# nmdp-bioinformatics/py-graph-imputation

Hardware: AMD Instinct MI355X
Metric: imputed subjects/sec (whole node), 5-locus CAU graph (higher is better)
Workload: dtype f64; 1 GPU; BASELINE configs[1]: CAU 5-locus graph, 10k synthetic fully-typed subjects; 10000 subjects per step and GPU, seed=rank; graph_nodes=35411, populations=1

## Files before the change

### py-graph-imputation_amd/csrc/grim_engine.hip

```cpp
#include <hip/hip_runtime.h>
#include <hip/hip_ext.h>
#include <stdio.h>
#include <stdlib.h>
#include <string.h>
#include <algorithm>
#include <atomic>
#include <mutex>
#include <string>
#include <vector>

#include "grim_plan_a.h"
#include "grim_plan_b.h"
#include "grim_small.h"
#include "grim_medium.h"
#include "grim_mid.h"
#include "grim_tables.h"
#include "grim_tokdev.h"
#include "grim_em.h"
#include "grim_engine_internal.h"
#include "grim_host_internal.h"
#include "grim_sdma.h"

__global__ __launch_bounds__(GRIM_WG, GRIM_WG_PER_CU) void grim_plan_a_kernel(DevArgs A) {
  __shared__ WgShared sh;
  __shared__ WaveTop wt[GRIM_NWAVE];
  const int tid = threadIdx.x;
  const int P = A.g.P;
  Slot S = make_slot(A, blockIdx.x);
  const uint32_t n_bail = A.bail_list ? A.queue[5] : 0, n_bail_heavy = A.bail_list ? A.queue[7] : 0;
  const uint32_t n_mid = A.mid_list ? A.queue[17] : 0;
  if (tid < GRIM_NWAVE * 4) ((unsigned long long *)sh.wctr)[tid] = 0;
  wg_arena(sh, wt);
// ... 186 lines not shown
  if (threadIdx.x == 0) pending = after_plan_b ? 0u : queue[2] + queue[6] + queue[9] + queue[10];
  for (int i = threadIdx.x; i < GRIM_NCTR + GRIM_NQ / 2; i += blockDim.x) host_state[i] = state[i];
  __syncthreads();
  if (pending) return;
  for (int i = threadIdx.x; i < GRIM_NCTR; i += blockDim.x) state[i] = 0;
  if (threadIdx.x < GRIM_NQ) ((uint32_t *)(state + GRIM_NCTR))[threadIdx.x] = threadIdx.x == 1 ? row_head0 : 0u;
}

struct grim_ctx {
  int device;
  hipStream_t stream;
  hipStream_t copy_stream;
  hipStream_t up_stream;
  GrimSdma *sdma;
  int export_mode;
  std::mutex err_mu;
  std::string err;
  std::mutex run_mu;
  int n_cu;
  void *scratch;
  uint64_t scratch_bytes;
  uint32_t *wctr;
  std::vector<grim_batch *> spare;
};

struct grim_graph {
  grim_ctx *ctx;
  DevGraph d;
  std::vector<void *> bufs;
  uint64_t bytes;
// ... 88 lines not shown
#define HIPCHK(call, ctxp, ret)                                                        \
  do {                                                                                 \
    hipError_t e_ = (call);                                                            \
    if (e_ != hipSuccess) {                                                            \
      set_err((ctxp), std::string(#call) + ": " + hipGetErrorString(e_));             \
      return ret;                                                                      \
    }                                                                                  \
  } while (0)

extern "C" int grim_device_count(void) {
  int n = 0;
  if (hipGetDeviceCount(&n) != hipSuccess) return 0;
  return n;
}

extern "C" grim_ctx *grim_create(int device_id) {
  int n = 0;
  if (hipGetDeviceCount(&n) != hipSuccess || n <= 0) {
    g_err = "grim_create: no HIP device visible";
    return nullptr;
  }
  if (device_id < 0 || device_id >= n) {
    g_err = "grim_create: device id out of range";
    return nullptr;
  }
  grim_ctx *c = new grim_ctx();
  c->device = device_id;
  c->copy_stream = nullptr;
  c->up_stream = nullptr;
  if (hipSetDevice(device_id) != hipSuccess || hipStreamCreate(&c->stream) != hipSuccess ||
// ... 8 lines not shown
  c->scratch = nullptr;
  c->scratch_bytes = 0;
  c->wctr = nullptr;
  if (hipMalloc((void **)&c->wctr, 4 * GRIM_WCTR_WORDS) != hipSuccess) {
    (void)hipGetLastError();
    g_err = "grim_create: cannot allocate the work counters";
    hipStreamDestroy(c->stream);
    hipStreamDestroy(c->copy_stream);
    hipStreamDestroy(c->up_stream);
    delete c;
    return nullptr;
  }
  if (hipGetDeviceProperties(&prop, device_id) == hipSuccess) c->n_cu = prop.multiProcessorCount;
  c->sdma = nullptr;
  c->export_mode = 1;
  {
    const char *e = getenv("GRIM_EXPORT");
    int want = 2;
    if (e && !strcmp(e, "kernel")) want = 1;
    else if (e && !strcmp(e, "memcpy")) want = 0;
    else if (!e && getenv("GRIM_EXPORT_KERNEL")) want = atoi(getenv("GRIM_EXPORT_KERNEL")) ? 1 : 0;
    if (want == 2) {
      char bdf[64] = {0};
      const char *why = nullptr;
      if (hipDeviceGetPCIBusId(bdf, (int)sizeof(bdf), device_id) != hipSuccess) bdf[0] = 0;
      c->sdma = grim_sdma_open(bdf[0] ? bdf : nullptr, device_id, &why);
      if (c->sdma) {
        const size_t probe = 1500000;
        void *hp = nullptr, *dp = nullptr;
        char report[256];
// ... 176 lines not shown
static uint64_t align256(uint64_t x) { return (x + 255) & ~255ull; }

static thread_local int tl_device = -1;
static inline void use_device(int dev) {
  if (tl_device != dev) {
    hipSetDevice(dev);
    tl_device = dev;
  }
}

static int env_int(const char *name, int dflt) {
  const char *v = getenv(name);
  return v ? atoi(v) : dflt;
}

uint32_t engine_small_stride(const grim_params *p) { return GRIM_SMALL_ROWS_FIXED + (p->n_results < 16 ? p->n_results : 16); }

uint64_t engine_rows_per_subject(const grim_params *p, uint32_t P) {
  return 2ull * p->n_results + 2ull * (p->n_pop_results < (uint64_t)P * P ? p->n_pop_results : (uint64_t)P * P);
}

static bool dev_realloc(uint8_t *&ptr, uint64_t bytes) {
  if (ptr) hipFree(ptr);
  ptr = nullptr;
  return hipMalloc((void **)&ptr, bytes ? bytes : 256) == hipSuccess;
}
static bool pin_realloc(uint8_t *&ptr, uint64_t bytes) {
  if (ptr) hipHostFree(ptr);
  ptr = nullptr;
  return hipHostMalloc((void **)&ptr, bytes ? bytes : 256, hipHostMallocDefault) == hipSuccess;
}
// ... 370 lines not shown
  }
  b->dev_lo = ld->dev_lo;
  b->dev_hi = ld->dev_hi;
  b->n_dev_lines = ld->dev_hi > ld->dev_lo ? ld->dev_hi - ld->dev_lo : 0;
  b->n_irregular = 0;
  b->n_subj = ld->n_subj;
  b->n_small = ld->n_small;
  b->n_medium = ld->n_medium;
  b->n_general = ld->n_general;
  b->last_load = *ld;
  b->last_load.priors = nullptr;
  A.n_medium = ld->n_medium;
  A.n_work = ld->n_general;
  unsigned long long *hs = (unsigned long long *)b->h_in;
  memset(hs, 0, 8 * (GRIM_NCTR + GRIM_NQ / 2));
  {
    const uint64_t staged = ((uint64_t)b->n_small + b->n_dev_lines) * b->small_stride;
    A.row_cap = (uint32_t)(b->row_limit - (staged <= b->row_limit ? staged : 0));
  }
  const bool host_subjects = ld->n_small + ld->n_medium + ld->n_general > 0;
  const uint64_t bytes = (!host_subjects && b->n_dev_lines) ? b->off_subj : b->off_tok + 2 * ld->tok_used;
  HIPCHK(hipMemcpyAsync(b->d_in, b->h_in, bytes, hipMemcpyHostToDevice, c->up_stream), c, -1);
  HIPCHK(hipEventRecord(b->ev_up, c->up_stream), c, -1);
  b->up_pending = true;
  g_moved[0] += bytes;
  {
    uint64_t R = (1ull << 20) + 512ull * ((uint64_t)ld->n_medium + ld->n_general) + 16ull * ld->n_small;
    R += (uint64_t)(ld->n_general < 256u ? ld->n_general : 256u) * (A.pair_cap / 2);
    const char *env_pool = getenv("GRIM_PAIR_POOL");
    if (env_pool && atol(env_pool) > 0) R = (uint64_t)atol(env_pool);
    if (b->pool_want > R) R = b->pool_want;
    if (R > 0x7FFFFFF0ull) R = 0x7FFFFFF0ull;
    const uint64_t items = 2ull * ld->n_subj < R / 256 + 1 ? 2ull * ld->n_subj : R / 256 + 1;
    uint64_t cap_b = R / 4 + (items + 1) * ((uint64_t)P * P + 4), cap_u = R / 4 + items * 64 + 1024;
// ... 17 lines not shown
    }
    b->pool_cap = R;
    A.ppool = (PairRec *)(b->d_pool + o_pool);
    A.ppool_cap = (uint32_t)R;
    A.taux = (TabAux *)(b->d_pool + o_aux);
    A.tboff = (uint32_t *)(b->d_pool + o_boff);
    A.tcell = (CellRec *)(b->d_pool + o_cell);
    A.tboff_cap = (uint32_t)cap_b;
    A.tunits = (TabUnit *)(b->d_pool + o_units);
    A.tunits_cap = (uint32_t)cap_u;
    A.tstride = (uint32_t)R;
    A.psort = (uint32_t *)(b->d_pool + o_sort);
    A.pgrp = (GrpRec *)(b->d_pool + o_grp);
    A.pprob = (double *)(b->d_pool + o_prob);
  }
  const uint32_t per_block = GRIM_WG / 32;
  b->n_host_small_waves = ((b->n_small + per_block - 1) / per_block) * (GRIM_WG / 64);
  b->n_small_waves = b->n_host_small_waves + ((b->n_dev_lines + per_block - 1) / per_block) * (GRIM_WG / 64);
  uint32_t slots = (uint32_t)c->n_cu * GRIM_WG_PER_CU;
  static const int env_slots = env_int("GRIM_SLOTS", 0);
  if (env_slots > 0) slots = (uint32_t)env_slots;
  if (slots > ld->n_subj) slots = ld->n_subj;
  if (slots == 0) slots = 1;
  b->n_slots = slots;
  b->scratch_need = (uint64_t)A.lay.stride * slots;
  if (b->gexec) {
    hipGraphExecDestroy(b->gexec);
    b->gexec = nullptr;
  }
  b->graph_state = 0;
  b->rows_used = 0;
  b->small_ctr_pending = false;
  return 0;
// ... 122 lines not shown
  launch(b, PH_NONE, grim_tables_merge_wave_kernel, dim3(g5), dim3(64), A);
  launch_span(b, PH_TABLES, false, true, grim_tables_merge_kernel, dim3(g2), dim3(GRIM_WG), A);
}

static void enqueue_half_wave(grim_batch *b, bool timed, const DevArgs &Ak, const SmallRec *recs, const uint32_t *order, uint32_t n, uint32_t stage) {
  const uint32_t per_block = GRIM_WG / 32;
  launch(b, timed ? PH_HALF_WAVE : PH_NONE, grim_plan_a_small_kernel, dim3((n + per_block - 1) / per_block), dim3(GRIM_WG), Ak, recs, n, stage,
         b->small_stride);
  launch(b, timed ? PH_COMPACT : PH_NONE, grim_small_compact_kernel, dim3((n + 63) / 64), dim3(64), b->a, order, order ? nullptr : recs, n, stage,
         b->small_stride);
}

static int enqueue_stage1(grim_batch *b) {
  grim_ctx *c = b->ctx;
  DevArgs &A = b->a;
  const uint32_t stage0 = (uint32_t)b->row_limit - (b->n_small + b->n_dev_lines) * b->small_stride;
  if (b->n_small) enqueue_half_wave(b, b->n_dev_lines == 0, A, b->d_small, b->d_os, b->n_small, stage0);
  if (b->n_dev_lines) {
    DevTok T;
    T.text = b->d_text;
    T.lines = b->d_lines;
    T.lo = b->dev_lo;
    T.hi = b->dev_hi;
    T.dict = b->dict->d;
    T.dsmall = b->d_dsmall;
    T.subj = const_cast<grim_subject *>(A.subj);
    T.tok = const_cast<uint16_t *>(A.tok);
    T.tok_base = (uint32_t)(b->plan.tok_cap ? b->plan.tok_cap : 1);
    T.graph_loci = A.g.n_loci;
    const dim3 tgrid((b->n_dev_lines + (GRIM_WG / 64) * TOK_LINES_PER_WAVE - 1) / ((GRIM_WG / 64) * TOK_LINES_PER_WAVE));
    launch(b, PH_TOKENIZER, grim_tokenize_kernel, tgrid, dim3(GRIM_WG), A, T);
    DevArgs A2 = A;
    A2.small_ctr = A.small_ctr + 2 * b->n_host_small_waves;
    enqueue_half_wave(b, true, A2, b->d_dsmall, nullptr, b->n_dev_lines, stage0 + b->n_small * b->small_stride);
  }
  if (b->n_medium) {
    static const int waves_per_cu = env_int("GRIM_MEDIUM_WAVES", GRIM_MEDIUM_WAVES_PER_CU);
    uint32_t grid = (uint32_t)c->n_cu * (uint32_t)(waves_per_cu > 0 ? waves_per_cu : GRIM_MEDIUM_WAVES_PER_CU);
    if (grid > b->n_medium) grid = b->n_medium;
    launch(b, PH_ONE_WAVE, grim_plan_a_medium_kernel, dim3(grid), dim3(64), A, b->d_om, b->n_medium, A.bail_list);
  }
  if (A.mid_list && b->n_general + b->n_medium) {
    const uint32_t want = b->n_general + b->n_medium;
    uint32_t grid = (uint32_t)c->n_cu * GRIM_MID_WG_PER_CU;
    if (grid > want) grid = want;
    launch(b, PH_MID, grim_plan_a_mid_kernel, dim3(grid), dim3(GRIM_WG), A);
  }
  if (b->n_general + b->n_medium) {
    uint32_t want = b->n_general + b->n_medium;
// ... 11 lines not shown
  return 0;
}

int engine_batch_upload_done(grim_batch *b) {
  if (!b || !b->up_pending) return 1;
  use_device(b->ctx->device);
  if (hipEventQuery(b->ev_up) == hipSuccess) return 1;
  (void)hipGetLastError();
  return 0;
}

int engine_batch_enqueue(grim_batch *b) {
  if (!b) return -1;
  grim_ctx *c = b->ctx;
  use_device(c->device);
  if (((uint64_t)b->n_small + b->n_dev_lines) * b->small_stride > b->row_limit) {
    b->rows_used = 0;
    set_err(c, "grim_batch_run: output row pool smaller than the half-wave kernel's fixed region");
    return -2;
  }
  memset(b->ms, 0, sizeof(b->ms));
  b->launched = 0;
  std::lock_guard<std::mutex> lk(c->run_mu);
  if (bind_scratch(b) != 0) return -1;
  if (b->up_pending) {
    b->up_pending = false;
    if (hipEventQuery(b->ev_up) != hipSuccess) {
      (void)hipGetLastError();
      HIPCHK(hipStreamWaitEvent(c->stream, b->ev_up, 0), c, -1);
    }
  }
  if (b->timing) {
    if (enqueue_stage1(b) != 0) {
      set_err(c, "grim_batch_run: kernel launch failed");
      return -1;
// ... 616 lines not shown
```

### py-graph-imputation_amd/csrc/grim_layout.h

```cpp
#pragma once
#include <stdint.h>

#include "../../include/grim_hip.h"

struct SmallRec {
  uint16_t tok[2 * GRIM_MAXL];
  uint8_t slot[GRIM_MAXL];
  uint8_t same;
  uint16_t prior_idx;
  uint32_t si;
};

struct PairRec {
  uint64_t k1, k2;
  double prob;
  uint32_t e1, e2;
};

struct TabWork {
  uint32_t si, n, off, mask;
};
#define GRIM_TAB_T1_MAX 256
struct TabAux {
  uint32_t boff[2];
// ... 7 lines not shown
  double sum;
  uint32_t head, pad;
};
struct CellRec {
  double sum;
  uint32_t first, pad;
};
struct TabUnit {
  uint32_t item, tb;
  uint32_t off;
  uint32_t lo, n;
  uint32_t pad[3];
};

#define GRIM_SMALL_ROWS_FIXED 1

enum { GRIM_CLS_SMALL = 0, GRIM_CLS_MEDIUM = 1, GRIM_CLS_GENERAL = 2 };

struct ClassRule {
  bool small_ok;
  bool medium_ok;
  double medium_max_cost;
  uint32_t graph_loci;
  uint64_t opt_threshold;
};

static inline double grim_cost(const grim_subject &sj);
static inline int grim_classify(const ClassRule &R, const grim_subject &sj) {
  bool sm = R.small_ok && sj.n_loci == GRIM_MAXL && R.graph_loci == GRIM_MAXL && sj.flags == 0;
  for (int l = 0; l < GRIM_MAXL && sm; ++l) sm = sj.cnt[l][0] == 1 && sj.cnt[l][1] == 1 && sj.wid[l][0] == 1 && sj.wid[l][1] == 1;
// ... 30 lines not shown
```

### py-graph-imputation_amd/csrc/grim_small.h

```cpp
#pragma once
#include "grim_pair.h"


__device__ __forceinline__ double half_shfl_d(double v, int src_in_half) {
  return __shfl(v, (threadIdx.x & 32) | src_in_half);
}
__device__ __forceinline__ uint32_t half_shfl_u(uint32_t v, int src_in_half) {
  return __shfl(v, (threadIdx.x & 32) | src_in_half);
}

template <int CTRL>
__device__ __forceinline__ double dpp_d(double v) {
  const long long b = __double_as_longlong(v);
  const int lo = __builtin_amdgcn_update_dpp(0, (int)(uint32_t)b, CTRL, 0xF, 0xF, false);
  const int hi = __builtin_amdgcn_update_dpp(0, (int)(uint32_t)((unsigned long long)b >> 32), CTRL, 0xF, 0xF, false);
  return __longlong_as_double((long long)(((unsigned long long)(uint32_t)hi << 32) | (uint32_t)lo));
}
__device__ __forceinline__ double row16_max(double v) {
  double o;
  o = dpp_d<0x121>(v); v = o > v ? o : v;
  o = dpp_d<0x122>(v); v = o > v ? o : v;
  o = dpp_d<0x124>(v); v = o > v ? o : v;
  o = dpp_d<0x128>(v); v = o > v ? o : v;
  return v;
}

__global__ __launch_bounds__(GRIM_WG) void grim_plan_a_small_kernel(DevArgs A, const SmallRec *recs, uint32_t n,
                                                                   uint32_t row_base, uint32_t row_stride) {
  const DevGraph &g = A.g;
  const int hl = threadIdx.x & 31;
  const uint32_t w = blockIdx.x * (GRIM_WG / 32) + (threadIdx.x >> 5);
  bool live = w < n;
  const int n_ladder = A.prm.n_ladder;
  double lad[8];
#pragma unroll
  for (int i = 0; i < 8; ++i) lad[i] = A.prm.ladder[i];
  bool hit = false;
  uint64_t mykey = 0;
  double f = 0.0;
  uint32_t same = 0, si = 0;
  double w_prior = 0.0;
  if (live) {
    const uint4 *rp = (const uint4 *)(recs + w);
    const uint4 r0 = rp[0], r1 = rp[1];
    const uint32_t words[8] = {r0.x, r0.y, r0.z, r0.w, r1.x, r1.y, r1.z, r1.w};
    same = (words[6] >> 8) & 0xFFu;
    si = words[7];
    live = si != GRIM_NONE;
    w_prior = live ? A.priors[(uint64_t)(words[6] >> 16)] : 0.0;
#pragma unroll
    for (int l = 0; l < GRIM_MAXL; ++l) {
      const uint32_t tw = words[l];
      const uint32_t t = ((hl >> l) & 1) ? (tw >> 16) : (tw & 0xFFFFu);
      const uint32_t slot = (l < 4 ? (words[5] >> (8 * l)) : words[6]) & 0xFFu;
      mykey |= (uint64_t)(t + 1u) << (GRIM_ABITS * slot);
    }
    uint32_t h = fht_hash(mykey) & g.fht_mask;
    for (; live;) {
      const FullEnt e = g.fht[h];
      if (e.key == mykey) { hit = true; f = e.f0; break; }
      if (e.key == 0) break;
      h = (h + 1) & g.fht_mask;
    }
  }
  const bool hit2 = half_shfl_u(hit ? 1u : 0u, hl ^ 31) != 0;
  const double f2 = half_shfl_d(f, hl ^ 31);
  const uint64_t key2 = ((uint64_t)half_shfl_u((uint32_t)(mykey >> 32), hl ^ 31) << 32) | half_shfl_u((uint32_t)mykey, hl ^ 31);
  const uint32_t het4 = 15u & ~same;
  bool kept = hl < 16 && ((uint32_t)hl & ~het4 & 15u) == 0 && (!((same >> 4) & 1u) || ((uint32_t)hl ^ het4) >= (uint32_t)hl);
  const bool pair_ok = live && kept && f > 0.0 && f2 > 0.0;
  const bool same_hap = mykey == key2;
  PairRef pr;
  pr.p1 = f; pr.p2 = f2; pr.m2 = f2;
  pr.e1 = same_hap ? 0u : 1u; pr.e2 = 0u;
  const bool hi_half = (threadIdx.x & 32) != 0;
  double eps = 0.0;
  bool found = false;
// ... 1 lines not shown
  {
    const uint64_t okb = __ballot(pair_ok);
    bool need_lo = (okb & 0xFFFFull) != 0, need_hi = ((okb >> 32) & 0xFFFFull) != 0;
    bool got_lo = false, got_hi = false;
    double eps_lo = 0.0, eps_hi = 0.0;
    auto step = [&](double e) {
      const bool a = pair_ok && pair_accept(e, pr, w_prior);
      const uint64_t b = __ballot(a);
      const bool take_lo = need_lo && (b & 0xFFFFull), take_hi = need_hi && ((b >> 32) & 0xFFFFull);
      if (take_lo) { need_lo = false; got_lo = true; eps_lo = e; }
      if (take_hi) { need_hi = false; got_hi = true; eps_hi = e; }
      if (hi_half ? take_hi : take_lo) acc = a;
    };
#pragma unroll
    for (int idx = 0; idx < 8; ++idx)
      if (idx < n_ladder && (need_lo || need_hi)) step(lad[idx]);
    for (int idx = 8; idx < n_ladder && (need_lo || need_hi); ++idx) step(A.prm.ladder[idx]);
    eps = hi_half ? eps_hi : eps_lo;
    found = hi_half ? got_hi : got_lo;
  }
  double prob = acc ? pair_prob(pr, w_prior) : 0.0;
  double mx = row16_max(prob);
  if (found && eps > 0.0) {
    eps = mx / 100000.0;
    acc = pair_ok && pair_accept(eps, pr, w_prior);
    prob = acc ? pair_prob(pr, w_prior) : 0.0;
    mx = row16_max(prob);
  }
  const uint64_t bal = __ballot(acc);
  const uint32_t accmask = (uint32_t)(hi_half ? (bal >> 32) : bal) & 0xFFFFu;
  const uint32_t nU = __popc(accmask);
  double total = 0.0;
  bool first = true;
  uint32_t rank = 0;
  for (uint32_t um = ((uint32_t)bal | (uint32_t)(bal >> 32)) & 0xFFFFu; um; um &= um - 1) {
    const int i = __builtin_ctz(um);
    const double p_lo = lane_get(prob, i), p_hi = lane_get(prob, 32 + i);
    const double pi = hi_half ? p_hi : p_lo;
    if ((accmask >> i) & 1u) {
      total = first ? pi : total + pi;
      first = false;
      if (pi > prob || (pi == prob && i < hl)) ++rank;
    }
  }
  {
    const uint64_t need = __ballot(live && kept), needp = __ballot(live && kept && hit),
                   needq = __ballot(live && kept && hit2);
    if ((threadIdx.x & 63) == 0) {
      const uint32_t gw = blockIdx.x * (GRIM_WG / 64) + (threadIdx.x >> 6);
      *(uint2 *)(A.small_ctr + 2 * gw) = make_uint2(2u * (uint32_t)__popcll(need), (uint32_t)(__popcll(needp) + __popcll(needq)));
    }
  }
  if (!live) return;
  const uint32_t off = row_base + w * row_stride;
  const bool ok = nU > 0;
  const int first_lane = ok ? (__ffs(accmask) - 1) : 0;
  const uint32_t n_pm = (ok && A.prm.out_haps) ? (nU < A.prm.n_results ? nU : A.prm.n_results) : 0;
  const uint64_t ka = ((uint64_t)half_shfl_u((uint32_t)(mykey >> 32), first_lane) << 32) | half_shfl_u((uint32_t)mykey, first_lane);
  const uint64_t kb = ((uint64_t)half_shfl_u((uint32_t)(key2 >> 32), first_lane) << 32) | half_shfl_u((uint32_t)key2, first_lane);
  {
    const int f = hl - 16;
    const bool phase = hl < 16;
    const bool wr = ok && (phase ? (acc && rank < n_pm) : f == 0);
    if (wr) {
      grim_row r;
      r.a = phase ? mykey : ka;
      r.b = phase ? key2 : kb;
      r.prob = phase ? prob : total;
      r.popa = 0;
      r.popb = 0;
      A.rows[off + (phase ? GRIM_SMALL_ROWS_FIXED + rank : (uint32_t)f)] = r;
    }
  }
  if (hl >= 19 && hl < 26) {
    const int j = hl - 19;
    const uint8_t status = ok ? GRIM_ST_OK : (A.prm.planb ? GRIM_ST_UNSUPPORTED : GRIM_ST_MISS);
    const uint32_t head = (uint32_t)status | ((uint32_t)'a' << 8) | ((!ok && A.prm.planb) ? (2u << 16) : 0u);
    const uint32_t n_um = (ok && A.prm.out_muug && A.prm.n_results) ? 1u : 0u;
    const uint32_t n_up = (ok && A.prm.out_muug && A.prm.n_pop_results) ? 1u : 0u;
    const uint32_t n_pp = (ok && A.prm.out_haps && A.prm.n_pop_results) ? 1u : 0u;
    const uint64_t mxb = ok ? (uint64_t)__double_as_longlong(mx) : 0ull;
    uint32_t lo, hi;
    switch (j) {
      case 0: lo = head; hi = ok ? nU : 0u; break;
      case 1: lo = ok ? 1u : 0u; hi = ok ? off + 0 : 0u; break;
      case 2: lo = ok ? off + 0 : 0u; hi = ok ? off + GRIM_SMALL_ROWS_FIXED : 0u; break;
      case 3: lo = ok ? off + 0 : 0u; hi = n_um; break;
      case 4: lo = n_up; hi = n_pm; break;
      case 5: lo = n_pp; hi = 0u; break;
      default: lo = (uint32_t)mxb; hi = (uint32_t)(mxb >> 32); break;
    }
    ((uint2 *)(A.res + si))[j] = make_uint2(lo, hi);
  }
  if (!ok && hl == 0 && A.prm.planb) push_next(A, si, false);
}
```

### py-graph-imputation_amd/csrc/grim_stream.cpp

```cpp
#include <errno.h>
#include <execinfo.h>
#include <fcntl.h>
#include <signal.h>
#include <sched.h>
#include <hip/hip_runtime_api.h>
#include <stdint.h>
#include <stdio.h>
#include <stdlib.h>
#include <string.h>
#include <sys/stat.h>
#include <sys/types.h>
#include <unistd.h>
#if defined(__x86_64__)
#include <immintrin.h>
#endif

#include <algorithm>
#include <atomic>
#include <chrono>
#include <condition_variable>
#include <deque>
#include <memory>
#include <mutex>
#include <string>
// ... 147 lines not shown
  grim_ctx *ctx = nullptr;
  const grim_graph *graph = nullptr;
  grim_params prm;
  grim_stream_opts opt;
  DictSnap snap;
  StreamRaces races;
  MaskTable masks;
  bool have_masks = false;
  ClassRule rule;
  FmtParams fp;
  uint32_t n_pops = 0;
  uint32_t chunk_lines = 0, granule = 1024, n_threads = 1, depth = 0;
  uint64_t rows_per_chunk = 0;
  grim_devdict *devdict = nullptr;
  bool dev_tok = false;
  std::atomic<uint64_t> rows_hint{0};
  uint64_t rows_max = 0;
  std::atomic<uint64_t> pool_hint{0};
  uint32_t cur_segment = 0;
  std::vector<std::array<uint64_t, 7>> seg_end;
  std::vector<uint8_t> seg_set;
  struct SegBuf {
    int k;
    char *p;
    size_t n;
    uint64_t rel;
  };
  struct PlacedWrite {
    int k;
    char *p;
// ... 185 lines not shown
      ld.text_bytes = c->text.size();
    }
    static const double one = 1.0;
    if (!s->races.n) {
      ld.n_priors = 0;
      ld.priors = &one;
    }
    lrc = engine_batch_load(b, &ld);
  }
  g_dbg_ns[0] += (uint64_t)(secs(tp0, tp1) * 1e9);
  g_dbg_ns[1] += (uint64_t)(secs(tp1, Clock::now()) * 1e9);
  return lrc;
}

static void part_stats(grim_stream *s, grim_batch *b, PartStats &ps) {
  if (!s->opt.timing) return;
  static_assert(sizeof(ps.kernel_ms) == sizeof(grim_stream_stats::kernel_ms), "kernel_ms: seven slots, GRIM_MS_TOTAL .. GRIM_MS_TABLES");
  for (int w = GRIM_MS_TOTAL; w <= GRIM_MS_TABLES; ++w) ps.kernel_ms[w] += grim_batch_kernel_ms(b, w);
  uint64_t ctr[4];
  if (grim_batch_counters(b, ctr) == 0)
    for (int k = 0; k < 4; ++k) ps.counters[k] += ctr[k];
}

static int device_part_sync(grim_stream *s, Chunk *c, uint32_t lo, uint32_t hi, bool whole, PartStats &ps);

static int fixup_part(grim_stream *s, Chunk *c, uint32_t lo, uint32_t hi, PartStats &ps) {
  grim_batch *b = c->batch;
  const uint32_t nrows1 = grim_batch_total_rows(b);
  const size_t base1 = c->extra_rows.size();
  c->extra_rows.resize(base1 + nrows1);
  if (engine_batch_fetch(b, lo, hi, nrows1 ? c->extra_rows.data() + base1 : nullptr) != 0) return -1;
  const EngineHost *H = engine_batch_host(b);
  grim_subject_result *res = H->res;
// ... 1233 lines not shown
  s->chunk_lines = opts->chunk_lines ? opts->chunk_lines : 131072u;
  s->granule = 1024;
  if (s->chunk_lines < s->granule) s->granule = s->chunk_lines;
  s->depth = opts->depth ? opts->depth : 4u;
  int nt = opts->n_threads;
  if (nt <= 0) nt = (int)grim_default_threads();
  s->n_threads = (uint32_t)nt;
  const uint64_t per = engine_rows_per_subject(prm, n_pops);
  uint64_t rows = opts->rows_per_chunk ? opts->rows_per_chunk : 32ull * s->chunk_lines;
  const uint64_t floor_rows = 2ull * engine_small_stride(prm) * s->chunk_lines + 2 * per + 4 * 64 + 1024;
  if (rows < floor_rows && !(opts->rows_exact && opts->rows_per_chunk)) rows = floor_rows;
  if (rows > 0x7FFFFFF0ull) rows = 0x7FFFFFF0ull;
  s->rows_per_chunk = rows;
  s->rows_max = opts->rows_per_chunk ? 0 : std::max<uint64_t>(rows, std::min<uint64_t>(0x7FFFFFF0ull, floor_rows + per * s->chunk_lines));
  {
    const char *e = getenv("GRIM_DEVICE_TOKENIZER");
    s->dev_tok = s->rule.small_ok && !s->have_masks && s->snap.n_loci == GRIM_MAXL && !(e && atoi(e) == 0);
    if (s->dev_tok) {
      s->devdict = engine_devdict_create(ctx, &s->snap);
      if (!s->devdict) {
        delete s;
        return nullptr;
      }
    }
  }
  EnginePlan plan0{s->chunk_lines, (uint64_t)s->chunk_lines * 48, s->dev_tok ? (uint64_t)s->chunk_lines * 128 : 0ull};
  for (uint32_t i = 0; i < s->depth; ++i) {
    std::unique_ptr<Chunk> c(new Chunk());
    c->slot_no = (int)i;
    c->batch = engine_batch_create(ctx, g, prm, rows, &plan0);
// ... 98 lines not shown
```

### py-graph-imputation_amd/csrc/grim_tokdev.h

```cpp
#pragma once
#include "grim_dev.h"
#include "grim_tok.h"

struct DevTok {
  const uint8_t *text;
  const LineRec *lines;
  uint32_t lo, hi;
  DevDict dict;
  SmallRec *dsmall;
  grim_subject *subj;
  uint16_t *tok;
  uint32_t tok_base;
  uint32_t graph_loci;
};
#define GRIM_REASON_HOST_TOKENIZER 7
#define GRIM_Q_IRREGULAR 18

#define TOK_LANES (2 * GRIM_MAXL)
#define TOK_LINES_PER_WAVE (64 / TOK_LANES)

__global__ __launch_bounds__(GRIM_WG) void grim_tokenize_kernel(DevArgs A, DevTok T) {
  const int lane = lane_id();
  const int a = lane % TOK_LANES, lw = lane / TOK_LANES;
  const uint32_t idx = (blockIdx.x * (GRIM_WG / 64) + wave_id()) * TOK_LINES_PER_WAVE + lw;
  const uint32_t line = T.lo + idx;
  const bool in_grid = lw < TOK_LINES_PER_WAVE && line < T.hi;
  LineRec lr;
  lr.gl_off = 0; lr.gl_len = 0; lr.prior_idx = 0;
  if (in_grid) lr = T.lines[line];
  const bool active = in_grid && lr.gl_len != 0;
  bool bad = active && lr.gl_len > GRIM_TOK_MAXGL;
  const uint32_t n = (active && !bad) ? lr.gl_len : 0;
  __shared__ uint4 lbuf[GRIM_WG / 64][TOK_LINES_PER_WAVE + 1][TOK_LANES];
  uint4 *mybuf = lbuf[wave_id()][lw < TOK_LINES_PER_WAVE ? lw : TOK_LINES_PER_WAVE];
  const uint32_t a0 = lr.gl_off & ~15u, skip = lr.gl_off - a0, tot = n ? skip + n : 0;
  uint4 q = make_uint4(0, 0, 0, 0);
  if (16u * (uint32_t)a < tot) q = ((const uint4 *)(T.text + a0))[a];
  mybuf[a] = q;
  uint32_t m_sep = 0, m_plus = 0;
  {
    const uint32_t wd[4] = {q.x, q.y, q.z, q.w};
#pragma unroll
    for (int bb = 0; bb < 16; ++bb) {
      const uint32_t pos = 16u * (uint32_t)a + (uint32_t)bb;
      const uint32_t c = (wd[bb >> 2] >> (8 * (bb & 3))) & 0xFFu;
      const bool in = pos >= skip && pos < tot;
      if (in && c == '+') m_plus |= 1u << bb;
      if (in && (c == '+' || c == '^')) m_sep |= 1u << bb;
// ... 98 lines not shown
    for (int k = 0; k < GRIM_MAXL; ++k) {
      const int src = base + 2 * k;
      const int sk = __shfl(slot, src < 64 ? src : 0);
      const int ek = __shfl(eq ? 1 : 0, src < 64 ? src : 0);
      if (sk >= 0) {
        used |= 1u << sk;
        slots5 |= (uint32_t)sk << (4 * k);
      }
      same |= (uint32_t)(ek & 1) << k;
    }
  }
  const uint64_t badm = __ballot(bad);
  const uint32_t line_bad = (uint32_t)(badm >> base) & ((1u << TOK_LANES) - 1u);
  const bool ok = active && line_bad == 0 && __popc(used) == GRIM_MAXL && T.graph_loci == GRIM_MAXL && T.dict.n_loci == GRIM_MAXL;
  if (!in_grid) return;
  SmallRec *rec = T.dsmall + idx;
  if (ok) {
    rec->tok[a] = (uint16_t)id;
    T.tok[(uint64_t)T.tok_base + (uint64_t)TOK_LANES * line + a] = (uint16_t)id;
    if ((a & 1) == 0) rec->slot[a >> 1] = (uint8_t)slot;
  }
  if (a == 0) {
    if (ok) {
      rec->same = (uint8_t)same;
      rec->prior_idx = lr.prior_idx;
      rec->si = line;
      grim_subject sj;
      sj.tok_off = T.tok_base + TOK_LANES * line;
      sj.prior_idx = lr.prior_idx;
      sj.n_loci = GRIM_MAXL;
      sj.flags = 0;
// ... 5 lines not shown
      }
      sj.pad[0] = (uint8_t)same;
      sj.pad[1] = sj.pad[2] = 0;
      sj.reserved[0] = sj.reserved[1] = 0;
      T.subj[line] = sj;
    } else {
      rec->si = GRIM_NONE;
      if (active) {
        uint32_t *r = (uint32_t *)(A.res + line);
        r[0] = (uint32_t)GRIM_ST_UNSUPPORTED | ((uint32_t)'a' << 8) | ((uint32_t)GRIM_REASON_HOST_TOKENIZER << 16);
        atomicAdd(A.queue + GRIM_Q_IRREGULAR, 1u);
      }
    }
  }
}
```

Before: 180.6 million subjects/s.

## Fuse device tokenizer and small-subject scoring into one chunk kernel

Adds a fused kernel that tokenizes device lines into LDS records, scores them in the same workgroup with the first hash-table probe issued early for all rounds, and writes rows compactly via a workgroup prefix sum and one atomic row reservation. This replaces the separate tokenize kernel plus half-wave small kernel, removing a launch and the global round-trip of SmallRec records, and no longer reserves a fixed per-subject staging stride for device lines. It adds an atomic on the row head per workgroup and a larger LDS footprint that may lower occupancy. It is enabled by default but disabled when timing is on.

```diff
diff --git a/py-graph-imputation_amd/csrc/grim_chunk.h b/py-graph-imputation_amd/csrc/grim_chunk.h
--- /dev/null
+++ b/py-graph-imputation_amd/csrc/grim_chunk.h
@@ -0,0 +1,97 @@
+#pragma once
+#include "grim_small.h"
+#include "grim_tokdev.h"
+
+#define CHUNK_ROUNDS (TOK_LINES_PER_WAVE / 2)
+#define CHUNK_ROWS_MAX (GRIM_SMALL_ROWS_FIXED + GRIM_SMALL_PM_MAX)
+#define CHUNK_HDR_PIECES ((int)(sizeof(grim_subject_result) / 8))
+#define CHUNK_COPY_LANES (GRIM_WG / TOK_LINES_PER_WG)
+
+struct ChunkShared {
+  TokLineBuf lbuf[GRIM_WG / 64];
+  SmallRec rec[TOK_LINES_PER_WG];
+  grim_row rows[TOK_LINES_PER_WG][CHUNK_ROWS_MAX];
+  uint2 hdr[TOK_LINES_PER_WG][CHUNK_HDR_PIECES];
+  uint32_t cnt[TOK_LINES_PER_WG];
+  uint32_t pre[TOK_LINES_PER_WG];
+  uint32_t base;
+  uint32_t fits;
+};
+static_assert(TOK_LINES_PER_WAVE % 2 == 0, "a round is two records");
+static_assert(TOK_LINES_PER_WG <= 64, "one wave takes the prefix over the workgroup's row counts");
+static_assert(sizeof(SmallRec) == 32 && sizeof(grim_row) == 32 && sizeof(grim_subject_result) == 8 * 7, "layouts the copies below rely on");
+static_assert(offsetof(ChunkShared, rec) % 16 == 0 && offsetof(ChunkShared, rows) % 16 == 0, "16-byte LDS reads");
+static_assert(sizeof(ChunkShared) <= 24 * 1024, "several workgroups per CU");
+
+__global__ __launch_bounds__(GRIM_WG) void grim_chunk_kernel(DevArgs A, DevTok T) {
+  __shared__ ChunkShared sh;
+  const int tid = threadIdx.x, wv = wave_id(), lane = lane_id();
+  const SmallLadder L = small_ladder(A);
+  if (lane < TOK_LINES_PER_WAVE) sh.rec[wv * TOK_LINES_PER_WAVE + lane].si = GRIM_NONE;
+  tokenize_block(A, T, sh.rec, sh.lbuf);
+  WAVE_SYNC();
+  const int half = (tid >> 5) & 1, hl = tid & 31;
+  SmallCand c[CHUNK_ROUNDS];
+  FullEnt e[CHUNK_ROUNDS];
+#pragma unroll
+  for (int r = 0; r < CHUNK_ROUNDS; ++r) c[r] = small_key(A, &sh.rec[wv * TOK_LINES_PER_WAVE + 2 * r + half], true);
+#pragma unroll
+  for (int r = 0; r < CHUNK_ROUNDS; ++r) {
+    e[r].key = 0;
+    e[r].f0 = 0.0;
+    if (c[r].live) e[r] = A.g.fht[c[r].h];
+  }
+  uint32_t probes = 0, hits = 0;
+#pragma unroll
+  for (int r = 0; r < CHUNK_ROUNDS; ++r) {
+    const int k = wv * TOK_LINES_PER_WAVE + 2 * r + half;
+    const SmallOut o = small_score(A, L, c[r], e[r], sh.rows[k], sh.hdr[k], 0u);
+    probes += o.probes;
+    hits += o.hits;
+    if (hl == 0) sh.cnt[k] = o.n_rows;
+  }
+  if (lane == 0) *(uint2 *)(A.small_ctr + 2 * (blockIdx.x * (GRIM_WG / 64) + wv)) = make_uint2(probes, hits);
+  __syncthreads();
+  if (wv == 0) {
+    const uint32_t n = lane < TOK_LINES_PER_WG ? sh.cnt[lane] : 0u;
+    uint32_t incl = n;
+    for (int d = 1; d < 64; d <<= 1) {
+      const uint32_t o = __shfl_up(incl, d);
+      if (lane >= d) incl += o;
+    }
+    if (lane < TOK_LINES_PER_WG) sh.pre[lane] = incl - n;
+    if (lane == 63) {
+      const uint32_t total = incl;
+      uint32_t base = 0, fits = 1;
+      if (total) {
+        base = atomicAdd(A.row_head, total);
+        if ((uint64_t)base + total > A.row_cap) {
+          atomicExch(&A.counters[4], 1ull);
+          fits = 0;
+        }
+      }
+      sh.base = base;
+      sh.fits = fits;
+    }
+  }
+  __syncthreads();
+  const uint32_t base = sh.base;
+  if (sh.fits && tid < CHUNK_COPY_LANES * TOK_LINES_PER_WG) {
+    const int k = tid / CHUNK_COPY_LANES, q = tid % CHUNK_COPY_LANES;
+    const uint32_t n16 = 2 * sh.cnt[k];
+    const uint4 *sp = (const uint4 *)sh.rows[k];
+    uint4 *dp = (uint4 *)(A.rows + base + sh.pre[k]);
+    for (uint32_t i = q; i < n16; i += CHUNK_COPY_LANES) dp[i] = sp[i];
+  }
+  if (tid < CHUNK_HDR_PIECES * TOK_LINES_PER_WG) {
+    const int k = tid / CHUNK_HDR_PIECES, j = tid % CHUNK_HDR_PIECES;
+    const uint32_t si = sh.rec[k].si;
+    if (si != GRIM_NONE) {
+      uint2 v = sh.hdr[k][j];
+      const uint32_t delta = sh.cnt[k] ? base + sh.pre[k] : 0u;
+      if (j == 2 || j == 3) v.x += delta;
+      if (j == 1 || j == 2) v.y += delta;
+      ((uint2 *)(A.res + si))[j] = v;
+    }
+  }
+}
diff --git a/py-graph-imputation_amd/csrc/grim_engine.hip b/py-graph-imputation_amd/csrc/grim_engine.hip
--- a/py-graph-imputation_amd/csrc/grim_engine.hip
+++ b/py-graph-imputation_amd/csrc/grim_engine.hip
@@ -16,6 +16,7 @@
 #include "grim_mid.h"
 #include "grim_tables.h"
 #include "grim_tokdev.h"
+#include "grim_chunk.h"
 #include "grim_em.h"
 #include "grim_engine_internal.h"
 #include "grim_host_internal.h"
@@ -232,6 +233,7 @@
   hipStream_t up_stream;
   GrimSdma *sdma;
   int export_mode;
+  bool chunk_fused;
   std::mutex err_mu;
   std::string err;
   std::mutex run_mu;
@@ -350,6 +352,8 @@
   return n;
 }
 
+static int env_int(const char *name, int dflt);
+
 extern "C" grim_ctx *grim_create(int device_id) {
   int n = 0;
   if (hipGetDeviceCount(&n) != hipSuccess || n <= 0) {
@@ -388,6 +392,7 @@
   if (hipGetDeviceProperties(&prop, device_id) == hipSuccess) c->n_cu = prop.multiProcessorCount;
   c->sdma = nullptr;
   c->export_mode = 1;
+  c->chunk_fused = env_int("GRIM_CHUNK_FUSED", 1) != 0;
   {
     const char *e = getenv("GRIM_EXPORT");
     int want = 2;
@@ -594,7 +599,24 @@
   return v ? atoi(v) : dflt;
 }
 
-uint32_t engine_small_stride(const grim_params *p) { return GRIM_SMALL_ROWS_FIXED + (p->n_results < 16 ? p->n_results : 16); }
+uint32_t engine_small_stride(const grim_params *p) {
+  return GRIM_SMALL_ROWS_FIXED + (p->n_results < GRIM_SMALL_PM_MAX ? p->n_results : GRIM_SMALL_PM_MAX);
+}
+
+static bool chunk_fused(const grim_batch *b) { return b->n_dev_lines != 0 && !b->timing && b->ctx->chunk_fused; }
+
+static uint64_t staged_rows(const grim_batch *b) {
+  return ((uint64_t)b->n_small + (chunk_fused(b) ? 0u : b->n_dev_lines)) * b->small_stride;
+}
+
+static void batch_bind_run(grim_batch *b) {
+  const uint64_t staged = staged_rows(b);
+  b->a.row_cap = (uint32_t)(b->row_limit - (staged <= b->row_limit ? staged : 0));
+  const uint32_t per_block = GRIM_WG / 32;
+  b->n_host_small_waves = ((b->n_small + per_block - 1) / per_block) * (GRIM_WG / 64);
+  const uint32_t dev_blocks = chunk_fused(b) ? (b->n_dev_lines + TOK_LINES_PER_WG - 1) / TOK_LINES_PER_WG : (b->n_dev_lines + per_block - 1) / per_block;
+  b->n_small_waves = b->n_host_small_waves + dev_blocks * (GRIM_WG / 64);
+}
 
 uint64_t engine_rows_per_subject(const grim_params *p, uint32_t P) {
   return 2ull * p->n_results + 2ull * (p->n_pop_results < (uint64_t)P * P ? p->n_pop_results : (uint64_t)P * P);
@@ -995,10 +1017,7 @@
   A.n_work = ld->n_general;
   unsigned long long *hs = (unsigned long long *)b->h_in;
   memset(hs, 0, 8 * (GRIM_NCTR + GRIM_NQ / 2));
-  {
-    const uint64_t staged = ((uint64_t)b->n_small + b->n_dev_lines) * b->small_stride;
-    A.row_cap = (uint32_t)(b->row_limit - (staged <= b->row_limit ? staged : 0));
-  }
+  batch_bind_run(b);
   const bool host_subjects = ld->n_small + ld->n_medium + ld->n_general > 0;
   const uint64_t bytes = (!host_subjects && b->n_dev_lines) ? b->off_subj : b->off_tok + 2 * ld->tok_used;
   HIPCHK(hipMemcpyAsync(b->d_in, b->h_in, bytes, hipMemcpyHostToDevice, c->up_stream), c, -1);
@@ -1046,9 +1065,6 @@
     A.pgrp = (GrpRec *)(b->d_pool + o_grp);
     A.pprob = (double *)(b->d_pool + o_prob);
   }
-  const uint32_t per_block = GRIM_WG / 32;
-  b->n_host_small_waves = ((b->n_small + per_block - 1) / per_block) * (GRIM_WG / 64);
-  b->n_small_waves = b->n_host_small_waves + ((b->n_dev_lines + per_block - 1) / per_block) * (GRIM_WG / 64);
   uint32_t slots = (uint32_t)c->n_cu * GRIM_WG_PER_CU;
   static const int env_slots = env_int("GRIM_SLOTS", 0);
   if (env_slots > 0) slots = (uint32_t)env_slots;
@@ -1201,7 +1217,7 @@
 static int enqueue_stage1(grim_batch *b) {
   grim_ctx *c = b->ctx;
   DevArgs &A = b->a;
-  const uint32_t stage0 = (uint32_t)b->row_limit - (b->n_small + b->n_dev_lines) * b->small_stride;
+  const uint32_t stage0 = (uint32_t)(b->row_limit - staged_rows(b));
   if (b->n_small) enqueue_half_wave(b, b->n_dev_lines == 0, A, b->d_small, b->d_os, b->n_small, stage0);
   if (b->n_dev_lines) {
     DevTok T;
@@ -1215,11 +1231,15 @@
     T.tok = const_cast<uint16_t *>(A.tok);
     T.tok_base = (uint32_t)(b->plan.tok_cap ? b->plan.tok_cap : 1);
     T.graph_loci = A.g.n_loci;
-    const dim3 tgrid((b->n_dev_lines + (GRIM_WG / 64) * TOK_LINES_PER_WAVE - 1) / ((GRIM_WG / 64) * TOK_LINES_PER_WAVE));
-    launch(b, PH_TOKENIZER, grim_tokenize_kernel, tgrid, dim3(GRIM_WG), A, T);
+    const dim3 tgrid((b->n_dev_lines + TOK_LINES_PER_WG - 1) / TOK_LINES_PER_WG);
     DevArgs A2 = A;
     A2.small_ctr = A.small_ctr + 2 * b->n_host_small_waves;
-    enqueue_half_wave(b, true, A2, b->d_dsmall, nullptr, b->n_dev_lines, stage0 + b->n_small * b->small_stride);
+    if (chunk_fused(b)) {
+      launch(b, PH_NONE, grim_chunk_kernel, tgrid, dim3(GRIM_WG), A2, T);
+    } else {
+      launch(b, PH_TOKENIZER, grim_tokenize_kernel, tgrid, dim3(GRIM_WG), A, T);
+      enqueue_half_wave(b, true, A2, b->d_dsmall, nullptr, b->n_dev_lines, stage0 + b->n_small * b->small_stride);
+    }
   }
   if (b->n_medium) {
     static const int waves_per_cu = env_int("GRIM_MEDIUM_WAVES", GRIM_MEDIUM_WAVES_PER_CU);
@@ -1261,11 +1281,12 @@
   if (!b) return -1;
   grim_ctx *c = b->ctx;
   use_device(c->device);
-  if (((uint64_t)b->n_small + b->n_dev_lines) * b->small_stride > b->row_limit) {
+  if (staged_rows(b) > b->row_limit) {
     b->rows_used = 0;
     set_err(c, "grim_batch_run: output row pool smaller than the half-wave kernel's fixed region");
     return -2;
   }
+  batch_bind_run(b);
   memset(b->ms, 0, sizeof(b->ms));
   b->launched = 0;
   std::lock_guard<std::mutex> lk(c->run_mu);
diff --git a/py-graph-imputation_amd/csrc/grim_layout.h b/py-graph-imputation_amd/csrc/grim_layout.h
--- a/py-graph-imputation_amd/csrc/grim_layout.h
+++ b/py-graph-imputation_amd/csrc/grim_layout.h
@@ -45,6 +45,7 @@
 };
 
 #define GRIM_SMALL_ROWS_FIXED 1
+#define GRIM_SMALL_PM_MAX 16
 
 enum { GRIM_CLS_SMALL = 0, GRIM_CLS_MEDIUM = 1, GRIM_CLS_GENERAL = 2 };
 
diff --git a/py-graph-imputation_amd/csrc/grim_small.h b/py-graph-imputation_amd/csrc/grim_small.h
--- a/py-graph-imputation_amd/csrc/grim_small.h
+++ b/py-graph-imputation_amd/csrc/grim_small.h
@@ -25,42 +25,78 @@
   return v;
 }
 
-__global__ __launch_bounds__(GRIM_WG) void grim_plan_a_small_kernel(DevArgs A, const SmallRec *recs, uint32_t n,
-                                                                   uint32_t row_base, uint32_t row_stride) {
+struct SmallLadder {
+  int n;
+  double lad[8];
+};
+__device__ __forceinline__ SmallLadder small_ladder(const DevArgs &A) {
+  SmallLadder L;
+  L.n = A.prm.n_ladder;
+#pragma unroll
+  for (int i = 0; i < 8; ++i) L.lad[i] = A.prm.ladder[i];
+  return L;
+}
+
+struct SmallCand {
+  bool live;
+  uint64_t mykey;
+  uint32_t same, si, h;
+  double w_prior;
+};
+
+__device__ __forceinline__ SmallCand small_key(const DevArgs &A, const SmallRec *rec, bool live) {
   const DevGraph &g = A.g;
   const int hl = threadIdx.x & 31;
-  const uint32_t w = blockIdx.x * (GRIM_WG / 32) + (threadIdx.x >> 5);
-  bool live = w < n;
-  const int n_ladder = A.prm.n_ladder;
-  double lad[8];
-#pragma unroll
-  for (int i = 0; i < 8; ++i) lad[i] = A.prm.ladder[i];
-  bool hit = false;
-  uint64_t mykey = 0;
-  double f = 0.0;
-  uint32_t same = 0, si = 0;
-  double w_prior = 0.0;
+  SmallCand c;
+  c.live = live;
+  c.mykey = 0;
+  c.same = 0;
+  c.si = 0;
+  c.h = 0;
+  c.w_prior = 0.0;
   if (live) {
-    const uint4 *rp = (const uint4 *)(recs + w);
+    const uint4 *rp = (const uint4 *)rec;
     const uint4 r0 = rp[0], r1 = rp[1];
     const uint32_t words[8] = {r0.x, r0.y, r0.z, r0.w, r1.x, r1.y, r1.z, r1.w};
-    same = (words[6] >> 8) & 0xFFu;
-    si = words[7];
-    live = si != GRIM_NONE;
-    w_prior = live ? A.priors[(uint64_t)(words[6] >> 16)] : 0.0;
+    c.same = (words[6] >> 8) & 0xFFu;
+    c.si = words[7];
+    c.live = c.si != GRIM_NONE;
+    c.w_prior = c.live ? A.priors[(uint64_t)(words[6] >> 16)] : 0.0;
 #pragma unroll
     for (int l = 0; l < GRIM_MAXL; ++l) {
       const uint32_t tw = words[l];
       const uint32_t t = ((hl >> l) & 1) ? (tw >> 16) : (tw & 0xFFFFu);
       const uint32_t slot = (l < 4 ? (words[5] >> (8 * l)) : words[6]) & 0xFFu;
-      mykey |= (uint64_t)(t + 1u) << (GRIM_ABITS * slot);
-    }
-    uint32_t h = fht_hash(mykey) & g.fht_mask;
+      c.mykey |= (uint64_t)(t + 1u) << (GRIM_ABITS * slot);
+    }
+    c.h = fht_hash(c.mykey) & g.fht_mask;
+  }
+  return c;
+}
+
+struct SmallOut {
+  uint32_t n_rows;
+  uint32_t probes, hits;
+};
+
+__device__ __forceinline__ SmallOut small_score(const DevArgs &A, const SmallLadder &L, const SmallCand &c, FullEnt e, grim_row *rows, uint2 *hdr,
+                                                uint32_t off) {
+  const DevGraph &g = A.g;
+  const int hl = threadIdx.x & 31;
+  const bool live = c.live;
+  const int n_ladder = L.n;
+  const uint64_t mykey = c.mykey;
+  const uint32_t same = c.same, si = c.si;
+  const double w_prior = c.w_prior;
+  bool hit = false;
+  double f = 0.0;
+  {
+    uint32_t h = c.h;
     for (; live;) {
-      const FullEnt e = g.fht[h];
       if (e.key == mykey) { hit = true; f = e.f0; break; }
       if (e.key == 0) break;
       h = (h + 1) & g.fht_mask;
+      e = g.fht[h];
     }
   }
   const bool hit2 = half_shfl_u(hit ? 1u : 0u, hl ^ 31) != 0;
@@ -92,7 +128,7 @@
     };
 #pragma unroll
     for (int idx = 0; idx < 8; ++idx)
-      if (idx < n_ladder && (need_lo || need_hi)) step(lad[idx]);
+      if (idx < n_ladder && (need_lo || need_hi)) step(L.lad[idx]);
     for (int idx = 8; idx < n_ladder && (need_lo || need_hi); ++idx) step(A.prm.ladder[idx]);
     eps = hi_half ? eps_hi : eps_lo;
     found = hi_half ? got_hi : got_lo;
@@ -121,16 +157,15 @@
       if (pi > prob || (pi == prob && i < hl)) ++rank;
     }
   }
+  SmallOut out;
+  out.n_rows = 0;
   {
     const uint64_t need = __ballot(live && kept), needp = __ballot(live && kept && hit),
                    needq = __ballot(live && kept && hit2);
-    if ((threadIdx.x & 63) == 0) {
-      const uint32_t gw = blockIdx.x * (GRIM_WG / 64) + (threadIdx.x >> 6);
-      *(uint2 *)(A.small_ctr + 2 * gw) = make_uint2(2u * (uint32_t)__popcll(need), (uint32_t)(__popcll(needp) + __popcll(needq)));
-    }
-  }
-  if (!live) return;
-  const uint32_t off = row_base + w * row_stride;
+    out.probes = 2u * (uint32_t)__popcll(need);
+    out.hits = (uint32_t)(__popcll(needp) + __popcll(needq));
+  }
+  if (!live) return out;
   const bool ok = nU > 0;
   const int first_lane = ok ? (__ffs(accmask) - 1) : 0;
   const uint32_t n_pm = (ok && A.prm.out_haps) ? (nU < A.prm.n_results ? nU : A.prm.n_results) : 0;
@@ -147,7 +182,7 @@
       r.prob = phase ? prob : total;
       r.popa = 0;
       r.popb = 0;
-      A.rows[off + (phase ? GRIM_SMALL_ROWS_FIXED + rank : (uint32_t)f)] = r;
+      rows[phase ? GRIM_SMALL_ROWS_FIXED + rank : (uint32_t)f] = r;
     }
   }
   if (hl >= 19 && hl < 26) {
@@ -168,7 +203,30 @@
       case 5: lo = n_pp; hi = 0u; break;
       default: lo = (uint32_t)mxb; hi = (uint32_t)(mxb >> 32); break;
     }
-    ((uint2 *)(A.res + si))[j] = make_uint2(lo, hi);
+    hdr[j] = make_uint2(lo, hi);
   }
   if (!ok && hl == 0 && A.prm.planb) push_next(A, si, false);
-}
+  {
+    const uint32_t n_um = (A.prm.out_muug && A.prm.n_results) ? 1u : 0u, n_up = (A.prm.out_muug && A.prm.n_pop_results) ? 1u : 0u,
+                   n_pp = (A.prm.out_haps && A.prm.n_pop_results) ? 1u : 0u;
+    out.n_rows = (ok && (n_um | n_up | n_pm | n_pp)) ? GRIM_SMALL_ROWS_FIXED + n_pm : 0u;
+  }
+  return out;
+}
+
+__global__ __launch_bounds__(GRIM_WG) void grim_plan_a_small_kernel(DevArgs A, const SmallRec *recs, uint32_t n,
+                                                                   uint32_t row_base, uint32_t row_stride) {
+  const uint32_t w = blockIdx.x * (GRIM_WG / 32) + (threadIdx.x >> 5);
+  const SmallLadder L = small_ladder(A);
+  const SmallCand c = small_key(A, recs + w, w < n);
+  FullEnt e;
+  e.key = 0;
+  e.f0 = 0.0;
+  if (c.live) e = A.g.fht[c.h];
+  const uint32_t off = row_base + w * row_stride;
+  const SmallOut o = small_score(A, L, c, e, A.rows + off, (uint2 *)(A.res + c.si), off);
+  if ((threadIdx.x & 63) == 0) {
+    const uint32_t gw = blockIdx.x * (GRIM_WG / 64) + (threadIdx.x >> 6);
+    *(uint2 *)(A.small_ctr + 2 * gw) = make_uint2(o.probes, o.hits);
+  }
+}
diff --git a/py-graph-imputation_amd/csrc/grim_stream.cpp b/py-graph-imputation_amd/csrc/grim_stream.cpp
--- a/py-graph-imputation_amd/csrc/grim_stream.cpp
+++ b/py-graph-imputation_amd/csrc/grim_stream.cpp
@@ -185,6 +185,7 @@
   uint64_t rows_per_chunk = 0;
   grim_devdict *devdict = nullptr;
   bool dev_tok = false;
+  bool count_bytes = false;
   std::atomic<uint64_t> rows_hint{0};
   uint64_t rows_max = 0;
   std::atomic<uint64_t> pool_hint{0};
@@ -400,9 +401,10 @@
 }
 
 static void part_stats(grim_stream *s, grim_batch *b, PartStats &ps) {
-  if (!s->opt.timing) return;
+  if (!s->opt.timing && !s->count_bytes) return;
   static_assert(sizeof(ps.kernel_ms) == sizeof(grim_stream_stats::kernel_ms), "kernel_ms: seven slots, GRIM_MS_TOTAL .. GRIM_MS_TABLES");
-  for (int w = GRIM_MS_TOTAL; w <= GRIM_MS_TABLES; ++w) ps.kernel_ms[w] += grim_batch_kernel_ms(b, w);
+  if (s->opt.timing)
+    for (int w = GRIM_MS_TOTAL; w <= GRIM_MS_TABLES; ++w) ps.kernel_ms[w] += grim_batch_kernel_ms(b, w);
   uint64_t ctr[4];
   if (grim_batch_counters(b, ctr) == 0)
     for (int k = 0; k < 4; ++k) ps.counters[k] += ctr[k];
@@ -1666,6 +1668,8 @@
   s->rows_per_chunk = rows;
   s->rows_max = opts->rows_per_chunk ? 0 : std::max<uint64_t>(rows, std::min<uint64_t>(0x7FFFFFF0ull, floor_rows + per * s->chunk_lines));
   {
+    const char *cb = getenv("GRIM_STREAM_COUNTERS");
+    s->count_bytes = cb && atoi(cb) != 0;
     const char *e = getenv("GRIM_DEVICE_TOKENIZER");
     s->dev_tok = s->rule.small_ok && !s->have_masks && s->snap.n_loci == GRIM_MAXL && !(e && atoi(e) == 0);
     if (s->dev_tok) {
diff --git a/py-graph-imputation_amd/csrc/grim_tokdev.h b/py-graph-imputation_amd/csrc/grim_tokdev.h
--- a/py-graph-imputation_amd/csrc/grim_tokdev.h
+++ b/py-graph-imputation_amd/csrc/grim_tokdev.h
@@ -19,11 +19,14 @@
 #define TOK_LANES (2 * GRIM_MAXL)
 #define TOK_LINES_PER_WAVE (64 / TOK_LANES)
 
-__global__ __launch_bounds__(GRIM_WG) void grim_tokenize_kernel(DevArgs A, DevTok T) {
+#define TOK_LINES_PER_WG ((GRIM_WG / 64) * TOK_LINES_PER_WAVE)
+typedef uint4 TokLineBuf[TOK_LINES_PER_WAVE + 1][TOK_LANES];
+
+__device__ __forceinline__ void tokenize_block(const DevArgs &A, const DevTok &T, SmallRec *recs, TokLineBuf *lbuf) {
   const int lane = lane_id();
   const int a = lane % TOK_LANES, lw = lane / TOK_LANES;
-  const uint32_t idx = (blockIdx.x * (GRIM_WG / 64) + wave_id()) * TOK_LINES_PER_WAVE + lw;
-  const uint32_t line = T.lo + idx;
+  const uint32_t slot_k = wave_id() * TOK_LINES_PER_WAVE + lw;
+  const uint32_t line = T.lo + blockIdx.x * TOK_LINES_PER_WG + slot_k;
   const bool in_grid = lw < TOK_LINES_PER_WAVE && line < T.hi;
   LineRec lr;
   lr.gl_off = 0; lr.gl_len = 0; lr.prior_idx = 0;
@@ -31,7 +34,6 @@
   const bool active = in_grid && lr.gl_len != 0;
   bool bad = active && lr.gl_len > GRIM_TOK_MAXGL;
   const uint32_t n = (active && !bad) ? lr.gl_len : 0;
-  __shared__ uint4 lbuf[GRIM_WG / 64][TOK_LINES_PER_WAVE + 1][TOK_LANES];
   uint4 *mybuf = lbuf[wave_id()][lw < TOK_LINES_PER_WAVE ? lw : TOK_LINES_PER_WAVE];
   const uint32_t a0 = lr.gl_off & ~15u, skip = lr.gl_off - a0, tot = n ? skip + n : 0;
   uint4 q = make_uint4(0, 0, 0, 0);
@@ -160,7 +162,7 @@
   const uint32_t line_bad = (uint32_t)(badm >> base) & ((1u << TOK_LANES) - 1u);
   const bool ok = active && line_bad == 0 && __popc(used) == GRIM_MAXL && T.graph_loci == GRIM_MAXL && T.dict.n_loci == GRIM_MAXL;
   if (!in_grid) return;
-  SmallRec *rec = T.dsmall + idx;
+  SmallRec *rec = recs + slot_k;
   if (ok) {
     rec->tok[a] = (uint16_t)id;
     T.tok[(uint64_t)T.tok_base + (uint64_t)TOK_LANES * line + a] = (uint16_t)id;
@@ -196,3 +198,8 @@
     }
   }
 }
+
+__global__ __launch_bounds__(GRIM_WG) void grim_tokenize_kernel(DevArgs A, DevTok T) {
+  __shared__ TokLineBuf lbuf[GRIM_WG / 64];
+  tokenize_block(A, T, T.dsmall + blockIdx.x * TOK_LINES_PER_WG, lbuf);
+}
```

After: 165.7 million subjects/s. -8.2%, worse.
